# anilshanbhag/gpu-sort

Measured on AMD Instinct MI355X. Metric: Gkeys/s sorting 2^30 uint32 keys; achieved HBM GB/s vs roofline, higher is better.
Workload: dtype u32; 1 GPU; lsb_radix_sort_2^30_u32_uniform_keys_only; keys_per_gpu=1073741824, algorithm=lsb, distribution=uniform, parallelism=single

## Files before the change

### gpu-sort_amd/_lib.py

```python
import ctypes as C
import os

import torch

_HERE = os.path.dirname(os.path.abspath(__file__))
LIB_PATH = os.environ.get("GS_LIB_PATH", os.path.join(_HERE, "lib", "libgpusort.so"))
CSRC_DIR = os.path.join(_HERE, "csrc")
INCLUDE_DIR = os.path.join(os.path.dirname(_HERE), "include")

GS_KEY_U32, GS_KEY_I32, GS_KEY_F32, GS_KEY_U64, GS_KEY_I64, GS_KEY_F64 = 0, 1, 2, 3, 4, 5
GS_KEY_U8, GS_KEY_I8, GS_KEY_U16, GS_KEY_I16 = 6, 7, 8, 9
GS_KEY_F16, GS_KEY_BF16, GS_KEY_F8 = 10, 11, 12
GS_GEN_UNIFORM, GS_GEN_ZIPF, GS_GEN_ENTROPY_AND, GS_GEN_ENUMERATED = 0, 1, 2, 3

u64, i32, vp, sz = C.c_uint64, C.c_int, C.c_void_p, C.c_size_t
pp = C.POINTER(C.c_void_p)

SIGNATURES = {
    "gs_version": (i32, []),
    "gs_error_string": (C.c_char_p, [i32]),
    "gs_lsb_temp_bytes": (sz, [u64, i32]),
    "gs_lsb_sort_u32": (i32, [vp, sz, pp, pp, C.POINTER(i32), u64, i32, i32, i32, i32, vp]),
    "gs_lsb_copy_temp_bytes": (sz, [u64, i32]),
    "gs_lsb_sort_copy_u32": (i32, [vp, sz, vp, vp, vp, vp, u64, i32, i32, i32, i32, vp]),
    "gs_lsb_wide_temp_bytes": (sz, [u64, i32, i32]),
    "gs_lsb_sort_wide": (i32, [vp, sz, pp, pp, C.POINTER(i32), u64, i32, i32, i32, i32, i32, i32, vp]),
    "gs_lsb_any_temp_bytes": (sz, [u64, i32, i32]),
    "gs_lsb_sort_any": (i32, [vp, sz, vp, vp, vp, vp, u64, i32, i32, i32, i32, i32, vp]),
    "gs_lsb_narrow_temp_bytes": (sz, [u64, i32, i32]),
    "gs_lsb_sort_narrow": (i32, [vp, sz, vp, vp, vp, vp, u64, i32, i32, i32, i32, i32, vp]),
    "gs_lsb_narrow_tile": (C.c_uint32, [i32, i32]),
    "gs_lsb_geometry": (None, [u64, i32, C.POINTER(C.c_uint32), C.POINTER(C.c_uint32), C.POINTER(C.c_uint32)]),
    "gs_lsb_workspace_layout": (i32, [vp, u64, pp, pp, pp]),
    "gs_lsb_pipe_status": (i32, [vp, u64, C.POINTER(C.c_uint32), vp]),
    "gs_lsb_plan_status": (i32, [vp, u64, C.POINTER(C.c_uint32), vp]),
    "gs_lsb_plan_look_only": (i32, [vp, vp, vp, u64, i32, i32, vp]),
    "gs_lsb_plan_layout": (i32, [u64, C.POINTER(C.c_uint64)]),
    "gs_lsb_upsweep_u32": (i32, [vp, sz, vp, u64, i32, i32, i32, i32, vp]),
    "gs_lsb_scan_spine": (i32, [vp, sz, u64, vp]),
    "gs_lsb_downsweep_u32": (i32, [vp, sz, vp, vp, vp, vp, u64, i32, i32, i32, i32, i32, vp]),
    "gs_msb_temp_bytes": (sz, [u64, i32]),
    "gs_msb_sort_u32": (i32, [vp, sz, vp, vp, u64, vp, vp, pp, pp, i32, vp, i32]),
    "gs_msb_wide_temp_bytes": (sz, [u64, i32, i32]),
    "gs_msb_sort_wide": (i32, [vp, sz, vp, vp, u64, vp, vp, i32, i32, pp, pp, i32, vp, i32]),
    "gs_msb_large_temp_bytes": (sz, [u64, i32]),
    "gs_msb_sort_large_u32": (i32, [vp, sz, vp, vp, u64, vp, vp, i32, vp, i32]),
    "gs_msb_large_wide_temp_bytes": (sz, [u64, i32, i32]),
    "gs_msb_sort_large_wide": (i32, [vp, sz, vp, vp, u64, vp, vp, i32, i32, i32, vp, i32]),
    "gs_lsb_large_temp_bytes": (sz, [u64, i32, i32]),
    "gs_lsb_sort_large": (i32, [vp, sz, pp, pp, C.POINTER(i32), u64, i32, i32, i32, i32, i32, i32, vp]),
    "gs_lsb_narrow_large_temp_bytes": (sz, [u64, i32, i32]),
    "gs_lsb_sort_narrow_large": (i32, [vp, sz, vp, vp, vp, vp, u64, i32, i32, i32, i32, i32, vp]),
    "gs_topk_temp_bytes": (sz, [u64, u64, i32]),
    "gs_topk_u32": (i32, [vp, sz, vp, vp, vp, vp, u64, u64, i32, i32, vp]),
    "gs_topk_status": (i32, [vp, u64, u64, i32, C.POINTER(C.c_uint32), vp]),
    "gs_msb_census": (i32, [vp, u64, i32, vp, vp]),
    "gs_msb_wide_census": (i32, [vp, u64, i32, i32, vp, vp]),
    "gs_msb_capacities": (None, [u64, i32, C.POINTER(C.c_uint32), C.POINTER(C.c_uint32), C.POINTER(C.c_uint32)]),
    "gs_msb_classify_upto": (i32, [vp, sz, vp, vp, u64, i32, i32, vp]),
    "gs_msb_read_lists": (i32, [vp, u64, i32, i32, vp, C.c_uint32, C.POINTER(C.c_uint32), C.POINTER(C.POINTER(C.c_uint32)), C.c_uint32,
                                C.POINTER(C.c_uint32), vp]),
    "gs_segmented_temp_bytes": (sz, [u64, i32, C.c_uint32]),
    "gs_segmented_sort_u32": (i32, [vp, sz, pp, pp, C.POINTER(i32), u64, C.c_uint32, vp, vp, i32, i32, i32, i32, vp]),
    "gs_segmented_wide_temp_bytes": (sz, [u64, i32, i32, C.c_uint32]),
    "gs_segmented_sort_wide": (i32, [vp, sz, pp, pp, C.POINTER(i32), u64, C.c_uint32, vp, vp, i32, i32, i32, i32, i32, i32, vp]),
    "gs_segmented_narrow_temp_bytes": (sz, [u64, i32, i32, C.c_uint32]),
    "gs_segmented_sort_narrow": (i32, [vp, sz, pp, pp, C.POINTER(i32), u64, C.c_uint32, vp, vp, i32, i32, i32, i32, i32, vp]),
    "gs_segmented_narrow_cap": (C.c_uint32, [i32, i32]),
# ... 85 lines not shown
```

### gpu-sort_amd/csrc/gs_lsb_downsweep.inc

```
#ifndef GS_EXP_SLEEP_MODE
#define GS_EXP_SLEEP_MODE 0
#endif
#ifndef GS_EXP_SLEEP_MIN_TILES
#define GS_EXP_SLEEP_MIN_TILES 49152u
#endif
#ifndef GS_EXP_SLEEP_PAIRS
#define GS_EXP_SLEEP_PAIRS 0
#endif
template <bool HAS_VALUES, bool OFF64 = false>
struct DownsweepSmem {
    uint32_t whist[LSB_WAVES][RADIX];
#ifdef GS_EXP_ALLWAVE_KEYS
    uint16_t wbase[LSB_WAVES][RADIX];
#else
    uint16_t wbase[HAS_VALUES ? LSB_WAVES : 1][RADIX];
#endif
    std::conditional_t<OFF64, uint64_t, uint32_t> gbase[RADIX];
    uint32_t stage[LSB_TILE * (HAS_VALUES ? 2 : 1)];
    uint32_t dead;
};

#ifdef GS_EXP_PHASES
__device__ uint32_t gs_phase_buf[131072 * 16];
#define GS_PHASE(k)                                                                          \
    do {                                                                                     \
        const unsigned long long now_ = __builtin_amdgcn_s_memtime();                        \
        if (tid == 0 && t < 131072u) gs_phase_buf[t * 16 + (k)] = (uint32_t)(now_ - tprev_); \
        tprev_ = now_;                                                                       \
    } while (0)
#define GS_PHASE_WAIT(what) asm volatile("s_waitcnt " what ::: "memory")
#else
#define GS_PHASE(k) do { } while (0)
#define GS_PHASE_WAIT(what) do { } while (0)
#endif

constexpr uint32_t PIPE_SPIN_LIMIT = 1u << 18;

template <bool HAS_VALUES, bool TAIL, int TW, bool BIG, bool PIPE, bool OFF64 = false>
__device__ __forceinline__ void downsweep_tile(DownsweepSmem<HAS_VALUES, OFF64> &sm, const uint32_t t,
    const uint32_t *__restrict__ keys_in, uint32_t *__restrict__ keys_out, const uint32_t *__restrict__ vals_in,
    uint32_t *__restrict__ vals_out, const uint32_t *__restrict__ spine, const uint16_t *__restrict__ prefix16,
    const uint32_t *__restrict__ totals, const PassParams &p, const uint64_t *__restrict__ sc, uint32_t tag,
    uint32_t *__restrict__ error_word, const uint32_t tid_ = threadIdx.x, const uint64_t *__restrict__ dbase = nullptr)
{
#ifdef GS_EXP_ALLWAVE_KEYS
    constexpr bool ALLWAVE = true;
#else
    constexpr bool ALLWAVE = HAS_VALUES;
#endif

    [[maybe_unused]] const int tid = (int)tid_;
    const int lane = (int)(tid_ & 63u), w = (int)(tid_ >> 6);
    const uint32_t full_tiles = p.n / (uint32_t)LSB_TILE;
    auto tw_in = [&](uint32_t k) { return TW == 0 ? k : twiddle_in(k, TW == 2 ? p.f32_in : 0, p.xor_in); };
    auto tw_out = [&](uint32_t k) { return TW == 0 ? k : twiddle_out(k, TW == 2 ? p.f32_out : 0, p.xor_out); };
    uint32_t wbits = p.bits;
    asm volatile("" : "+v"(wbits));
    auto digit = [&](uint32_t k) { return __builtin_amdgcn_ubfe(k, p.shift, wbits); };

    uint32_t *my = sm.whist[w];
    const uint16_t *mybase = sm.wbase[w];
    const uint32_t wbase = (uint32_t)w * (WAVE * LSB_KPT) + lane;
    const uint32_t tail_valid = p.n - full_tiles * (uint32_t)LSB_TILE;
    (void)full_tiles;

#ifdef GS_EXP_PHASES
    unsigned long long tprev_ = __builtin_amdgcn_s_memtime();
    const unsigned long long t0_ = tprev_, r0_ = __builtin_amdgcn_s_memrealtime();
#endif
#ifdef GS_EXP_SLEEP_START
    __builtin_amdgcn_s_sleep(GS_EXP_SLEEP_START);
#endif
    if (!HAS_VALUES) __builtin_amdgcn_s_setprio(3);
    const uint64_t tile_base = (uint64_t)t * LSB_TILE;
    const uint32_t valid = TAIL ? tail_valid : (uint32_t)LSB_TILE;

    uint64_t scg[4] = {0, 0, 0, 0};
    const uint64_t *scrow = nullptr;
    if (PIPE && w == 0) {
        scrow = sc + (size_t)(t / LSB_CHUNK) * RADIX + 4 * lane;
#pragma unroll
        for (int q = 0; q < 4; ++q) scg[q] = ld_agent(scrow + q);
    }

    uint32_t key[LSB_KPT], val[HAS_VALUES ? LSB_KPT : 1], pos[LSB_KPT];
    {
        const uint32_t *kin = keys_in + tile_base;
        if (!TAIL) {
#pragma unroll
            for (int i = 0; i < LSB_KPT; ++i) key[i] = kin[wbase + i * WAVE];
        } else {
            const uint32_t pad = twiddle_out(0xffffffffu, TW == 2 ? p.f32_in : 0, TW ? p.xor_in : 0u);
#pragma unroll
            for (int i = 0; i < LSB_KPT; ++i) {
                const uint32_t idx = wbase + i * WAVE;
                key[i] = pad;
                if (idx < tail_valid) key[i] = kin[idx];
            }
        }
    }
    GS_PHASE(0);
#ifndef GS_EXP_RANK_PRIO
#define GS_EXP_RANK_PRIO 0
#endif
    if (!HAS_VALUES) __builtin_amdgcn_s_setprio(GS_EXP_RANK_PRIO);
    if (HAS_VALUES) {
        const uint32_t *vin = vals_in + tile_base;
#pragma unroll
        for (int i = 0; i < LSB_KPT; ++i) {
            const uint32_t idx = wbase + i * WAVE;
            val[i] = 0;
            if (!TAIL || idx < valid) val[i] = vin[idx];
        }
    }
    uint32_t dstart[4] = {0, 0, 0, 0};
    if constexpr (OFF64) {
        if (TAIL && w == 0) {
            const uint4 tot = reinterpret_cast<const uint4 *>(totals)[lane];
            dstart[0] = tot.x; dstart[1] = tot.y; dstart[2] = tot.z; dstart[3] = tot.w;
        }
    } else if (w == 0) {
        const uint4 tot = reinterpret_cast<const uint4 *>(totals)[lane];
        const uint32_t lane_sum = tot.x + tot.y + tot.z + tot.w;
        const uint32_t ex = wave_inclusive_scan(lane_sum) - lane_sum;
        dstart[0] = ex + (TAIL ? tot.x : 0u);
        dstart[1] = dstart[0] + (TAIL ? tot.y : tot.x);
        dstart[2] = dstart[1] + (TAIL ? tot.z : tot.y);
        dstart[3] = dstart[2] + (TAIL ? tot.w : tot.z);
    }

    uint32_t tbase[4] = {0, 0, 0, 0};
    if (!TAIL && !PIPE && w == 0) {
        const uint32_t *sp = spine + (uint32_t)(4 * lane) * p.grid + t / LSB_CHUNK;
        const uint2 pf = reinterpret_cast<const uint2 *>(prefix16 + (size_t)t * RADIX)[lane];
        tbase[0] = sp[0] + (pf.x & 0xffffu);
        tbase[1] = sp[p.grid] + (pf.x >> 16);
        tbase[2] = sp[2 * p.grid] + (pf.y & 0xffffu);
        tbase[3] = sp[3 * p.grid] + (pf.y >> 16);
    }

    if (PIPE && !TAIL && w == 0) {
        uint32_t spins = 0;
        bool gave_up = false;
        for (;;) {
            const bool ok = (uint32_t)(scg[0] >> 32) == tag && (uint32_t)(scg[1] >> 32) == tag &&
                            (uint32_t)(scg[2] >> 32) == tag && (uint32_t)(scg[3] >> 32) == tag;
            if (__builtin_amdgcn_ballot_w64(!ok) == 0) break;
            if (++spins > PIPE_SPIN_LIMIT) {
                if (lane == 0) atomicOr(error_word, 1u);
                gave_up = true;
                break;
            }
            __builtin_amdgcn_s_sleep(8);
#pragma unroll
            for (int q = 0; q < 4; ++q) scg[q] = ld_agent(scrow + q);
        }
        if (lane == 0) sm.dead = gave_up ? 1u : 0u;
        const uint64_t pf = ld_agent(reinterpret_cast<const uint64_t *>(prefix16 + (size_t)t * RADIX) + lane);
        tbase[0] = (uint32_t)scg[0] + (uint32_t)(pf & 0xffffu);
        tbase[1] = (uint32_t)scg[1] + (uint32_t)((pf >> 16) & 0xffffu);
        tbase[2] = (uint32_t)scg[2] + (uint32_t)((pf >> 32) & 0xffffu);
        tbase[3] = (uint32_t)scg[3] + (uint32_t)(pf >> 48);
    }

    auto publish_gbase = [&](const uint32_t (&ex)[4], const uint32_t (&run)[4]) {
// ... 21 lines not shown
            reinterpret_cast<uint4 *>(sm.gbase)[lane] = make_uint4(g[0], g[1], g[2], g[3]);
        }
    };

#pragma unroll
    for (int i = lane; i < RADIX; i += WAVE) my[i] = 0;
    GS_PHASE_WAIT("vmcnt(0)");
    GS_PHASE(1);
#pragma unroll
    for (int i = 0; i < LSB_KPT; ++i) key[i] = tw_in(key[i]);
    {
        uint32_t d_prev = 0, plo = 0, phi = 0;
#pragma unroll
        for (int i = 0; i <= LSB_KPT; ++i) {
            uint32_t d_cur = 0, clo = 0, chi = 0;
            if (i < LSB_KPT) {
                d_cur = digit(key[i]);
                match_digit(d_cur, clo, chi);
            }
            if (i > 0) {
                const uint32_t lower = count_lower(plo, phi);
                pos[i - 1] = my[d_prev] + lower;
                if (lower == 0)
                    __hip_atomic_fetch_add(&my[d_prev], (uint32_t)(__popc(plo) + __popc(phi)), __ATOMIC_RELAXED,
                                           __HIP_MEMORY_SCOPE_WAVEFRONT);
            }
            d_prev = d_cur; plo = clo; phi = chi;
        }
    }
#pragma unroll
    for (int i = 0; i < LSB_KPT; ++i) {
        asm volatile("" : "+v"(pos[i]), "+v"(key[i]));
    }
    GS_PHASE_WAIT("lgkmcnt(0)");
    GS_PHASE(2);
    __syncthreads();
    GS_PHASE(3);
    if (PIPE && !TAIL && sm.dead) return;

    if constexpr (ALLWAVE) {
        uint32_t run[4] = {0, 0, 0, 0}, below[4] = {0, 0, 0, 0};
#pragma unroll
        for (int j = 0; j < LSB_WAVES; ++j) {
            const uint4 x = reinterpret_cast<const uint4 *>(sm.whist[j])[lane];
            run[0] += x.x; run[1] += x.y; run[2] += x.z; run[3] += x.w;
            if (j < w) { below[0] += x.x; below[1] += x.y; below[2] += x.z; below[3] += x.w; }
        }
        const uint32_t lane_sum = run[0] + run[1] + run[2] + run[3];
        uint32_t ex[4];
        ex[0] = wave_inclusive_scan(lane_sum) - lane_sum;
        ex[1] = ex[0] + run[0];
        ex[2] = ex[1] + run[1];
        ex[3] = ex[2] + run[2];
        reinterpret_cast<uint2 *>(sm.wbase[w])[lane] =
            make_uint2((ex[0] + below[0]) | ((ex[1] + below[1]) << 16), (ex[2] + below[2]) | ((ex[3] + below[3]) << 16));
        if (w == 0) publish_gbase(ex, run);
    } else {
        if (w == 0) {
            uint32_t run[4] = {0, 0, 0, 0};
#pragma unroll
            for (int j = 0; j < LSB_WAVES; ++j) {
                const uint4 x = reinterpret_cast<const uint4 *>(sm.whist[j])[lane];
                run[0] += x.x; run[1] += x.y; run[2] += x.z; run[3] += x.w;
            }
            const uint32_t lane_sum = run[0] + run[1] + run[2] + run[3];
            uint32_t ex[4];
            ex[0] = wave_inclusive_scan(lane_sum) - lane_sum;
            ex[1] = ex[0] + run[0];
            ex[2] = ex[1] + run[1];
            ex[3] = ex[2] + run[2];
            publish_gbase(ex, run);
            asm volatile("" ::: "memory");
            uint4 e4 = make_uint4(ex[0] << 2, ex[1] << 2, ex[2] << 2, ex[3] << 2);
#pragma unroll
            for (int j = 0; j < LSB_WAVES; ++j) {
                const uint4 x = reinterpret_cast<const uint4 *>(sm.whist[j])[lane];
                reinterpret_cast<uint4 *>(sm.whist[j])[lane] = e4;
                e4.x += x.x << 2; e4.y += x.y << 2; e4.z += x.z << 2; e4.w += x.w << 2;
            }
        }
        __syncthreads();
    }
    GS_PHASE(4);

    {
        uint32_t wb[LSB_KPT];
#pragma unroll
        for (int i = 0; i < LSB_KPT; ++i) {
            const uint32_t d = digit(key[i]);
            wb[i] = ALLWAVE ? (uint32_t)mybase[d] : my[d];
        }
#pragma unroll
        for (int i = 0; i < LSB_KPT; ++i) {
            if (HAS_VALUES) {
                reinterpret_cast<uint2 *>(sm.stage)[pos[i] + wb[i]] = make_uint2(key[i], val[i]);
            } else if (ALLWAVE) {
                sm.stage[pos[i] + wb[i]] = key[i];
            } else {
                const uint32_t at = (pos[i] << 2) + wb[i];
                *reinterpret_cast<uint32_t *>(reinterpret_cast<char *>(sm.stage) + at) = key[i];
            }
        }
    }
    GS_PHASE_WAIT("lgkmcnt(0)");
    GS_PHASE(5);
    __syncthreads();
    GS_PHASE(6);
#ifndef GS_EXP_SLEEP
#define GS_EXP_SLEEP 32
#define GS_EXP_SLEEP_MODE_DEFAULT 0
#else
#define GS_EXP_SLEEP_MODE_DEFAULT GS_EXP_SLEEP_MODE
#endif
    if ((!HAS_VALUES || GS_EXP_SLEEP_PAIRS) && full_tiles >= GS_EXP_SLEEP_MIN_TILES) {
        [[maybe_unused]] const int ws = __builtin_amdgcn_readfirstlane(w);
#if GS_EXP_SLEEP_MODE_DEFAULT == 3
        if (ws & 1) __builtin_amdgcn_s_sleep(GS_EXP_SLEEP); else __builtin_amdgcn_s_sleep(GS_EXP_SLEEP_B);
#elif GS_EXP_SLEEP_MODE_DEFAULT == 4
        if (ws >= 4) __builtin_amdgcn_s_sleep(GS_EXP_SLEEP);
#elif GS_EXP_SLEEP_MODE_DEFAULT == 1
        if (ws & 1) __builtin_amdgcn_s_sleep(GS_EXP_SLEEP);
#elif GS_EXP_SLEEP_MODE_DEFAULT == 0
        __builtin_amdgcn_s_sleep(GS_EXP_SLEEP);
#endif
    }
#ifndef GS_EXP_STORE_PRIO
#define GS_EXP_STORE_PRIO 3
#endif
    if (!HAS_VALUES) __builtin_amdgcn_s_setprio(GS_EXP_STORE_PRIO);
#pragma unroll
    for (int i = 0; i < LSB_KPT; ++i) {
        const uint32_t slot = (uint32_t)w * (WAVE * LSB_KPT) + i * WAVE + lane;
        uint32_t k, v = 0;
// ... 41 lines not shown
```

### gpu-sort_amd/csrc/gs_lsb_plan.hip

```cpp
#include "gs_device.hpp"
#include "gs_lsb.hpp"
#include "gs_msb_tasks.hpp"
#ifndef GS_PLAN_N_MIN
#define GS_PLAN_N_MIN (1ull << 28)
#endif
#include <cstddef>
#include <cstdlib>
#include <cstring>
#include <type_traits>

namespace gs {

#include "gs_lsb_upsweep.inc"

#include "gs_lsb_downsweep.inc"

constexpr uint32_t PLAN_GROUPS = 65536;
constexpr uint32_t PLAN_WORDS = PLAN_GROUPS / 2;
constexpr uint32_t PLAN_PLANNED = 1u, PLAN_CLASSIC = 2u;
constexpr uint32_t PLAN_SKIP = 0xffffffffu;
constexpr int PLAN_LOOK_THREADS = 1024, PLAN_LOOK_WAVES = PLAN_LOOK_THREADS / WAVE, PLAN_LOOK_BATCH = 32;
constexpr uint32_t PLAN_LOOK_HALVES = PLAN_LOOK_WAVES / LSB_CHUNK;
static_assert(PLAN_LOOK_WAVES % LSB_CHUNK == 0, "a look workgroup takes whole chunks");
constexpr uint32_t PLAN_LOOK_MAX_GRID = MI355X_CUS;
constexpr uint32_t PLAN_BLOCKS = 128, PLAN_BLOCK_WORDS = PLAN_WORDS / PLAN_BLOCKS, PLAN_BLOCK_GROUPS = PLAN_GROUPS / PLAN_BLOCKS;
constexpr int PLAN_SORT_BITS = 16;
constexpr int PLAN_SKEW_LANES = 8;

struct PlanBlock {
    uint32_t route, max_group, nonempty, tasks[MSB_NCLASS], total;
    uint32_t shift[4];
    uint32_t ups_skip[4];
    MsbLevel level[2];
    uint32_t wg_bad[PLAN_LOOK_MAX_GRID];
    uint32_t blk_total[PLAN_BLOCKS], blk_max[PLAN_BLOCKS], blk_nonempty[PLAN_BLOCKS];
    uint32_t blk_class[PLAN_BLOCKS][MSB_NCLASS];
    uint32_t blk_class_base[PLAN_BLOCKS][MSB_NCLASS];
    uint32_t offsets[PLAN_GROUPS + 1];
};
static_assert(sizeof(MsbLevel) == 64 && offsetof(PlanBlock, level) == 64, "plan block layout");

__device__ __forceinline__ int plan_class_of(uint32_t size)
{
    return size <= msb_class_cap(0) ? 0 : size <= msb_class_cap(1) ? 1 : size <= msb_class_cap(2) ? 2 : 3;
}

__device__ __forceinline__ void look_add(uint32_t *tab, uint32_t *my, uint32_t g)
{
    const unsigned long long act = __builtin_amdgcn_ballot_w64(true);
    const uint32_t g0 = __builtin_amdgcn_readfirstlane(g);
    if (__builtin_amdgcn_ballot_w64(g == g0) == act) {
        if (count_lower_mask(act) == 0) {
            atomicAdd(&tab[g0 >> 1], (uint32_t)__popcll(act) << ((g0 & 1u) * 16u));
            atomicAdd(&my[g0 & 0xffu], (uint32_t)__popcll(act));
        }
    } else {
        atomicAdd(&tab[g >> 1], 1u << ((g & 1u) * 16u));
        atomicAdd(&my[g & 0xffu], 1u);
    }
}

__device__ __forceinline__ void look_add_skew(uint32_t *tab, uint32_t *my, uint32_t g, int lane)
{
    unsigned long long rest = ~0ull;
#pragma unroll
    for (int r = 0; r < 2; ++r) {
        if (rest == 0ull) break;
        const int lead = __builtin_amdgcn_readfirstlane(__builtin_ctzll(rest));
        const uint32_t g0 = (uint32_t)__builtin_amdgcn_readlane((int)g, lead);
        const unsigned long long m = __builtin_amdgcn_ballot_w64(g == g0) & rest;
        if (lane == lead) {
            atomicAdd(&tab[g0 >> 1], (uint32_t)__popcll(m) << ((g0 & 1u) * 16u));
// ... 115 lines not shown
    __syncthreads();
    if (tid == 0) plan->wg_bad[blockIdx.x] = sm.red[0] != sm.red[1] ? 1u : 0u;
}

__global__ __launch_bounds__(RADIX) void lsb_plan_reduce_kernel(const uint32_t *__restrict__ partial, PlanBlock *__restrict__ plan, uint32_t parts)
{
    __shared__ uint32_t scratch[8];
    __shared__ uint32_t red[2 + MSB_NCLASS];
    const uint32_t tid = threadIdx.x, wi = blockIdx.x * PLAN_BLOCK_WORDS + tid;
    if (tid < 2 + MSB_NCLASS) red[tid] = 0;
    uint32_t c0 = 0, c1 = 0;
#pragma unroll 8
    for (uint32_t g = 0; g < parts; ++g) {
        const uint32_t v = partial[(size_t)g * PLAN_WORDS + wi];
        c0 += v & 0xffffu;
        c1 += v >> 16;
    }
    uint32_t total = 0;
    const uint32_t ex = block_exclusive_scan_256(c0 + c1, scratch, &total);
    plan->offsets[2 * wi] = ex;
    plan->offsets[2 * wi + 1] = ex + c0;
    atomicMax(&red[0], c0 > c1 ? c0 : c1);
    if (c0) { atomicAdd(&red[1], 1u); atomicAdd(&red[2 + plan_class_of(c0)], 1u); }
    if (c1) { atomicAdd(&red[1], 1u); atomicAdd(&red[2 + plan_class_of(c1)], 1u); }
    __syncthreads();
    if (tid == 0) {
        plan->blk_total[blockIdx.x] = total;
        plan->blk_max[blockIdx.x] = red[0];
        plan->blk_nonempty[blockIdx.x] = red[1];
    }
    if (tid < MSB_NCLASS) plan->blk_class[blockIdx.x][tid] = red[2 + tid];
}

__global__ __launch_bounds__(RADIX) void lsb_plan_decide_kernel(PlanBlock *__restrict__ plan, uint32_t n, uint32_t parts)
{
    __shared__ uint32_t s_base, s_total, s_max, s_nz, s_cls[MSB_NCLASS], s_clsbase[MSB_NCLASS];
    const uint32_t tid = threadIdx.x, b = blockIdx.x;
    if (tid == 0) {
        uint32_t base = 0, total = 0, mx = 0, nz = 0;
        for (uint32_t i = 0; i < PLAN_BLOCKS; ++i) {
            if (i == b) base = total;
            total += plan->blk_total[i];
            const uint32_t m = plan->blk_max[i];
            mx = m > mx ? m : mx;
            nz += plan->blk_nonempty[i];
        }
        s_base = base; s_total = total; s_max = mx; s_nz = nz;
    } else if (tid <= MSB_NCLASS) {
        const uint32_t c = tid - 1u;
        uint32_t base = 0, total = 0;
        for (uint32_t i = 0; i < PLAN_BLOCKS; ++i) {
            if (i == b) base = total;
            total += plan->blk_class[i][c];
        }
        s_cls[c] = total; s_clsbase[c] = base;
    }
    const int any_bad = __syncthreads_or(tid < parts ? (int)plan->wg_bad[tid] : 0);
    const uint32_t g = b * PLAN_BLOCK_GROUPS + 2u * tid;
    plan->offsets[g] += s_base;
    plan->offsets[g + 1] += s_base;
    if (tid < MSB_NCLASS) plan->blk_class_base[b][tid] = s_clsbase[tid];
    if (b == 0 && tid == 0) {
        const bool planned = !any_bad && s_total == n && s_max <= msb_class_cap(MSB_NCLASS - 1);
        plan->route = planned ? PLAN_PLANNED : PLAN_CLASSIC;
        plan->max_group = s_max;
        plan->nonempty = s_nz;
        plan->total = s_total;
        MsbLevel l0{}, l1{};
        for (int c = 0; c < MSB_NCLASS; ++c) {
            plan->tasks[c] = planned ? s_cls[c] : 0u;
            l0.task_count[c] = planned ? s_cls[c] : 0u;
        }
        l0.keys = n;
        l1.packed = planned ? (1ull << 32) : 0ull;
        plan->level[0] = l0;
        plan->level[1] = l1;
        for (int q = 0; q < 4; ++q) {
            plan->shift[q] = planned ? (q < 2 ? 16u + 8u * (uint32_t)q : PLAN_SKIP) : 8u * (uint32_t)q;
            plan->ups_skip[q] = planned && q != 1 ? 1u : 0u;
        }
        plan->offsets[PLAN_GROUPS] = n;
    }
}

struct PlanLists { MsbTask *tasks[MSB_NCLASS]; uint32_t cap[MSB_NCLASS]; };
__global__ __launch_bounds__(PLAN_BLOCK_GROUPS) void lsb_plan_tasks_kernel(const PlanBlock *__restrict__ plan, PlanLists lists)
{
    __shared__ uint32_t wcnt[PLAN_BLOCK_GROUPS / WAVE][MSB_NCLASS];
    if (plan->route != PLAN_PLANNED) return;
    const uint32_t tid = threadIdx.x, g = blockIdx.x * PLAN_BLOCK_GROUPS + tid;
    const int w = wave_id(), lane = lane_id();
    const uint32_t off = plan->offsets[g], size = plan->offsets[g + 1] - off;
    const int cls = size ? plan_class_of(size) : -1;
    uint32_t lower = 0;
#pragma unroll
    for (int c = 0; c < MSB_NCLASS; ++c) {
        const unsigned long long m = __builtin_amdgcn_ballot_w64(cls == c);
        if (cls == c) lower = count_lower_mask(m);
        if (lane == 0) wcnt[w][c] = (uint32_t)__popcll(m);
    }
    __syncthreads();
    if (cls >= 0) {
        uint32_t idx = plan->blk_class_base[blockIdx.x][cls] + lower;
        for (int j = 0; j < w; ++j) idx += wcnt[j][cls];
        if (idx < lists.cap[cls]) lists.tasks[cls][idx] = MsbTask{off, size, (uint32_t)PLAN_SORT_BITS, 0u};
    }
}

template <bool PLAIN>
__global__ __launch_bounds__(LSB_THREADS, GS_EXP_UPS_WPE) void lsb_plan_upsweep_kernel(const uint32_t *__restrict__ keys,
                                                                       uint32_t *__restrict__ spine, uint16_t *__restrict__ prefix16,
                                                                       const uint32_t *__restrict__ slot_shift,
                                                                       const uint32_t *__restrict__ slot_ups_skip, PassParams p)
{
    __shared__ UpsweepSmem<false, false> sm;
    const uint32_t sh = *slot_shift;
    if (sh == PLAN_SKIP || *slot_ups_skip) return;
    p.shift = sh;
    upsweep_chunk<false, false, PLAIN>(sm, keys, chunk_of_block(blockIdx.x, p.grid), spine, prefix16, nullptr, nullptr, p, PipeParams{});
}

template <bool TAIL, int TW, bool BIG>
__global__ __launch_bounds__(LSB_THREADS, 6) void lsb_plan_downsweep_kernel(const uint32_t *__restrict__ keys_in, uint32_t *__restrict__ keys_out,
                                                                            const uint32_t *__restrict__ totals, const uint32_t *__restrict__ spine,
                                                                            const uint16_t *__restrict__ prefix16,
                                                                            const uint32_t *__restrict__ slot_shift, PassParams p)
{
    __shared__ __attribute__((aligned(16))) DownsweepSmem<false> sm;
    const uint32_t sh = *slot_shift;
    if (sh == PLAN_SKIP) return;
    p.shift = sh;
    const uint32_t full_tiles = p.n / (uint32_t)LSB_TILE;
    if (!TAIL && blockIdx.x >= full_tiles) return;
    const uint32_t t = TAIL ? full_tiles : tile_of_item_wide(blockIdx.x, full_tiles);
    downsweep_tile<false, TAIL, TW, BIG, false>(sm, t, keys_in, keys_out, nullptr, nullptr, spine, prefix16, totals, p, nullptr, 0u, nullptr);
}

static inline size_t align256(size_t x) { return (x + 255) & ~(size_t)255; }

static inline bool plan_enabled()
{
    static const bool v = [] { const char *e = getenv("GS_LSB_KEYS_PLAN"); return !(e && strcmp(e, "classic") == 0); }();
    return v;
}
constexpr uint64_t PLAN_N_MAX = (uint64_t)PLAN_GROUPS * 16620u;
constexpr uint64_t PLAN_N_FLOOR = 65536;
constexpr uint64_t PLAN_N_MIN = GS_PLAN_N_MIN;
static inline uint64_t plan_min_items()
{
    static const uint64_t v = [] {
        const char *e = getenv("GS_LSB_PLAN_MIN_ITEMS");
        if (!e) return PLAN_N_MIN;
        const uint64_t x = strtoull(e, nullptr, 10);
        return x < PLAN_N_FLOOR ? PLAN_N_FLOOR : x;
    }();
    return v;
}
static inline bool plan_has_block(uint64_t n) { return !lsb_pipe_enabled() && n >= plan_min_items(); }
static inline bool plan_size_ok(uint64_t n) { return plan_has_block(n) && n <= PLAN_N_MAX; }
static inline uint32_t plan_list_cap(uint64_t n, int c)
{
    const uint64_t m = c == 0 ? n : n / ((uint64_t)msb_class_cap(c - 1) + 1u) + 1u;
    return (uint32_t)(m < PLAN_GROUPS ? m : PLAN_GROUPS);
}
static inline size_t plan_lists_bytes(uint64_t n)
{
    size_t b = 0;
    for (int c = 0; c < MSB_NCLASS; ++c) b += (size_t)plan_list_cap(n, c) * sizeof(MsbTask);
    return b;
}
static inline size_t plan_block_offset(uint64_t n)
{
    const size_t a = lsb_temp_bytes(n), b = plan_lists_bytes(n);
    return align256(a > b ? a : b);
}
static inline size_t plan_temp_bytes(uint64_t n) { return plan_block_offset(n) + align256(sizeof(PlanBlock)); }

template <int TW, bool BIG>
static void launch_plan_downsweep(const uint32_t *kin, uint32_t *kout, const LsbWorkspace &ws, const uint32_t *slot_shift,
                                  const PassParams &p, hipStream_t s)
{
    hipLaunchKernelGGL((lsb_plan_downsweep_kernel<false, TW, BIG>), dim3(p.ds_grid), dim3(LSB_THREADS), 0, s, kin, kout, ws.totals,
                       ws.spine, ws.prefix16, slot_shift, p);
}

static int lsb_plan_slot(const uint32_t *kin, uint32_t *kout, const LsbWorkspace &ws, const uint32_t *slot_shift,
                         const uint32_t *slot_ups_skip, const PassParams &p, bool real, bool ups_real, hipStream_t s)
{
    {
        KernelTimer kt(ups_real ? GS_K_LSB_UPSWEEP : GS_K_OTHER, s);
        if (!p.f32_in && !p.xor_in)
            hipLaunchKernelGGL(lsb_plan_upsweep_kernel<true>, dim3(p.grid), dim3(LSB_THREADS), 0, s, kin, ws.spine, ws.prefix16, slot_shift,
                               slot_ups_skip, p);
        else
            hipLaunchKernelGGL(lsb_plan_upsweep_kernel<false>, dim3(p.grid), dim3(LSB_THREADS), 0, s, kin, ws.spine, ws.prefix16, slot_shift,
                               slot_ups_skip, p);
    }
    {
        if (const int e = lsb_scan_as(ws.spine, ws.totals, p.grid, s, real ? GS_K_LSB_SCAN : GS_K_OTHER)) return e;
    }
    {
        KernelTimer kt(real ? GS_K_LSB_DOWNSWEEP : GS_K_OTHER, s);
        if (p.n >= (uint32_t)LSB_TILE) {
            const int tw = (p.f32_in || p.f32_out) ? 2 : ((p.xor_in | p.xor_out) ? 1 : 0);
            const bool big = p.n > (1u << 30);
#define GS_PDS(TW_, BIG_) launch_plan_downsweep<TW_, BIG_>(kin, kout, ws, slot_shift, p, s)
            if (big) { if (tw == 2) GS_PDS(2, true); else if (tw == 1) GS_PDS(1, true); else GS_PDS(0, true); }
            else { if (tw == 2) GS_PDS(2, false); else if (tw == 1) GS_PDS(1, false); else GS_PDS(0, false); }
#undef GS_PDS
        }
        if (p.n % (uint32_t)LSB_TILE)
            hipLaunchKernelGGL((lsb_plan_downsweep_kernel<true, 2, true>), dim3(1), dim3(LSB_THREADS), 0, s, kin, kout, ws.totals,
                               (const uint32_t *)nullptr, (const uint16_t *)nullptr, slot_shift, p);
    }
    return (int)hipGetLastError();
}

static int lsb_plan_look(const uint32_t *keys, uint32_t *alt, const LsbWorkspace &ws, PlanBlock *plan, uint64_t n, const PassParams &tw,
                         hipStream_t s)
{
    const uint32_t parts = (uint32_t)(n / PLAN_WORDS < PLAN_LOOK_MAX_GRID ? n / PLAN_WORDS : PLAN_LOOK_MAX_GRID);
    const uint32_t chunks = lsb_make_params(n, 16, RADIX_BITS).grid;
    KernelTimer kt(GS_K_OTHER, s);
    hipLaunchKernelGGL(lsb_plan_look_kernel, dim3(parts), dim3(PLAN_LOOK_THREADS), 0, s, keys, alt, plan, ws.spine, ws.prefix16, (uint32_t)n,
                       chunks, tw.f32_in, tw.xor_in);
    hipLaunchKernelGGL(lsb_plan_reduce_kernel, dim3(PLAN_BLOCKS), dim3(RADIX), 0, s, alt, plan, parts);
    hipLaunchKernelGGL(lsb_plan_decide_kernel, dim3(PLAN_BLOCKS), dim3(RADIX), 0, s, plan, (uint32_t)n, parts);
    return (int)hipGetLastError();
}

int lsb_plan_sort(char *base, uint32_t *d_keys[2], int *selector, uint64_t n, int descending, int key_type, hipStream_t s)
{
    const LsbWorkspace ws = lsb_carve(base, n);
    char *lists_end = base + plan_block_offset(n);
    PlanBlock *plan = (PlanBlock *)lists_end;
    PlanLists lists;
    for (int c = MSB_NCLASS - 1; c >= 0; --c) {
        lists.cap[c] = plan_list_cap(n, c);
        lists_end -= (size_t)lists.cap[c] * sizeof(MsbTask);
        lists.tasks[c] = (MsbTask *)lists_end;
    }
    int sel = *selector, e;
    PassParams tw{};
    lsb_twiddle_masks(key_type, descending, true, true, tw);
    if ((e = lsb_plan_look(d_keys[sel], d_keys[sel ^ 1], ws, plan, n, tw, s))) return e;
    for (int slot = 0; slot < 4; ++slot) {
        PassParams p = lsb_make_params(n, 0, RADIX_BITS);
        lsb_twiddle_masks(key_type, descending, slot == 0, slot == 3, p);
        if ((e = lsb_plan_slot(d_keys[sel], d_keys[sel ^ 1], ws, &plan->shift[slot], &plan->ups_skip[slot], p, slot < 2, slot == 1, s))) return e;
        sel ^= 1;
    }
    {
        KernelTimer kt(GS_K_OTHER, s);
        hipLaunchKernelGGL(lsb_plan_tasks_kernel, dim3(PLAN_BLOCKS), dim3(PLAN_BLOCK_GROUPS), 0, s, plan, lists);
    }
    if ((e = (int)hipGetLastError())) return e;
    if ((e = msb_local_sorts_in_place(plan->level, lists.tasks, PLAN_GROUPS, PLAN_GROUPS, d_keys[sel], PLAN_SORT_BITS, n, tw.f32_out,
                                      tw.xor_out, s)))
        return e;
    *selector = sel;
    return hipSuccess;
}


bool lsb_plan_has_block(uint64_t n) { return plan_has_block(n); }
size_t lsb_plan_temp_bytes(uint64_t n) { return plan_temp_bytes(n); }
bool lsb_plan_applies(uint64_t n) { return plan_enabled() && plan_size_ok(n); }

}

using namespace gs;

extern "C" {

int gs_lsb_plan_status(void *d_temp, uint64_t num_items, uint32_t out[8], void *stream)
{
    GS_CLEAR_STALE_ERROR();
    if (!d_temp || !out || num_items >= (1ull << 32)) return hipErrorInvalidValue;
    memset(out, 0, 8 * sizeof(uint32_t));
    if (!plan_enabled() || !plan_size_ok(num_items)) return hipSuccess;
    const PlanBlock *plan = (const PlanBlock *)(gs_ws_base(d_temp) + plan_block_offset(num_items));
    hipError_t e = hipMemcpyAsync(out, plan, 8 * sizeof(uint32_t), hipMemcpyDeviceToHost, (hipStream_t)stream);
    if (e == hipSuccess) e = hipStreamSynchronize((hipStream_t)stream);
    return (int)e;
}

int gs_lsb_plan_look_only(void *d_temp, const void *d_keys, void *d_alt, uint64_t num_items, int key_type, int descending, void *stream)
{
    GS_CLEAR_STALE_ERROR();
    if (!d_temp || !d_keys || !d_alt || num_items >= (1ull << 32)) return hipErrorInvalidValue;
    if (!plan_enabled() || !plan_size_ok(num_items)) return hipErrorInvalidValue;
    char *base = gs_ws_base(d_temp);
    PassParams tw{};
    lsb_twiddle_masks(key_type, descending, true, true, tw);
    return lsb_plan_look((const uint32_t *)d_keys, (uint32_t *)d_alt, lsb_carve(base, num_items), (PlanBlock *)(base + plan_block_offset(num_items)),
                         num_items, tw, (hipStream_t)stream);
}

int gs_lsb_plan_layout(uint64_t num_items, uint64_t out[4])
{
    if (!out || num_items >= (1ull << 32) || !plan_enabled() || !plan_size_ok(num_items)) return hipErrorInvalidValue;
    char *base = (char *)(uintptr_t)GS_WS_ALIGN;
    const LsbWorkspace ws = lsb_carve(base, num_items);
    out[0] = (uint64_t)((char *)ws.spine - base);
    out[1] = (uint64_t)((char *)ws.prefix16 - base);
    out[2] = plan_block_offset(num_items);
    out[3] = lsb_make_params(num_items, 16, RADIX_BITS).grid;
    return hipSuccess;
}

}
```

### include/gpusort.h

```cpp
#ifndef GPUSORT_H_
#define GPUSORT_H_

#include <stddef.h>
#include <stdint.h>

#ifdef __cplusplus
extern "C" {
#endif

#define GS_VERSION 100

enum gs_key_type {
    GS_KEY_U32 = 0,
    GS_KEY_I32 = 1,
    GS_KEY_F32 = 2,
    GS_KEY_U64 = 3,
    GS_KEY_I64 = 4,
    GS_KEY_F64 = 5,
    GS_KEY_U8 = 6,
    GS_KEY_I8 = 7,
    GS_KEY_U16 = 8,
    GS_KEY_I16 = 9,
    GS_KEY_F16 = 10,
    GS_KEY_BF16 = 11,
    GS_KEY_F8 = 12
};

int         gs_version(void);
const char *gs_error_string(int err);


size_t gs_lsb_temp_bytes(uint64_t num_items, int has_values);

int gs_lsb_sort_u32(void *d_temp, size_t temp_bytes,
                    uint32_t *d_keys[2], uint32_t *d_vals[2], int *selector,
                    uint64_t num_items, int begin_bit, int end_bit,
                    int descending, int key_type, void *stream);

size_t gs_lsb_copy_temp_bytes(uint64_t num_items, int has_values);
int gs_lsb_sort_copy_u32(void *d_temp, size_t temp_bytes,
                         const uint32_t *d_keys_in, uint32_t *d_keys_out,
                         const uint32_t *d_vals_in, uint32_t *d_vals_out,
                         uint64_t num_items, int begin_bit, int end_bit,
                         int descending, int key_type, void *stream);

size_t gs_lsb_wide_temp_bytes(uint64_t num_items, int key_bytes, int val_bytes);
int gs_lsb_sort_wide(void *d_temp, size_t temp_bytes, void *d_keys[2], void *d_vals[2],
                     int *selector, uint64_t num_items, int key_bytes, int val_bytes,
                     int begin_bit, int end_bit, int descending, int key_type, void *stream);

void gs_lsb_geometry(uint64_t num_items, int has_values, uint32_t *grid, uint32_t *tile,
                     uint32_t *tiles_per_chunk);
int  gs_lsb_workspace_layout(void *d_temp, uint64_t num_items, uint32_t **d_spine,
                             uint32_t **d_totals, uint16_t **d_prefix16);
int  gs_lsb_pipe_status(void *d_temp, uint64_t num_items, uint32_t *h_status, void *stream);
int  gs_lsb_plan_status(void *d_temp, uint64_t num_items, uint32_t out[8], void *stream);
int  gs_lsb_plan_look_only(void *d_temp, const void *d_keys, void *d_alt, uint64_t num_items,
                           int key_type, int descending, void *stream);
int  gs_lsb_plan_layout(uint64_t num_items, uint64_t out[4]);
int  gs_lsb_upsweep_u32(void *d_temp, size_t temp_bytes, const uint32_t *d_keys_in,
                        uint64_t num_items, int shift, int bits, int descending,
                        int key_type_in, void *stream);
int  gs_lsb_scan_spine(void *d_temp, size_t temp_bytes, uint64_t num_items, void *stream);
int  gs_lsb_downsweep_u32(void *d_temp, size_t temp_bytes,
                          const uint32_t *d_keys_in, uint32_t *d_keys_out,
                          const uint32_t *d_vals_in, uint32_t *d_vals_out,
                          uint64_t num_items, int shift, int bits, int descending,
                          int key_type_in, int key_type_out, void *stream);

size_t gs_lsb_any_temp_bytes(uint64_t num_items, int key_type, int val_bytes);
int gs_lsb_sort_any(void *d_temp, size_t temp_bytes, const void *d_keys_in, void *d_keys_out,
                    const void *d_vals_in, void *d_vals_out, uint64_t num_items, int key_type, int val_bytes,
                    int begin_bit, int end_bit, int descending, void *stream);

size_t gs_lsb_narrow_temp_bytes(uint64_t num_items, int key_type, int val_bytes);
int gs_lsb_sort_narrow(void *d_temp, size_t temp_bytes, const void *d_keys_in, void *d_keys_out,
                       const void *d_vals_in, void *d_vals_out, uint64_t num_items, int key_type, int val_bytes,
                       int begin_bit, int end_bit, int descending, void *stream);
uint32_t gs_lsb_narrow_tile(int key_type, int val_bytes);


size_t gs_msb_temp_bytes(uint64_t num_items, int has_values);

int gs_msb_sort_u32(void *d_temp, size_t temp_bytes,
                    uint32_t *d_keys, uint32_t *d_vals, uint64_t num_items,
                    uint32_t *d_keys_alt, uint32_t *d_vals_alt,
                    uint32_t **d_sorted_keys, uint32_t **d_sorted_vals,
                    int key_type, void *stream, int synchronize);

// ... 127 lines not shown
```

Measured before the change: 147.5 Gkeys/s.

## Scatter second plan pass via per-digit-pair cursors instead of stable spine offsets

In the planned LSB path, the second pass can now run in a cursor mode. The plan's per-group offsets seed a cursor table, and each full tile whose keys share one upper digit claims output ranges with atomic adds instead of reading the spine/prefix bases. Tiles that straddle two upper digits, plus the tail, are listed and handled by a separate irregular kernel that scatters with wave-aggregated atomics. The upsweep for that pass is skipped in cursor mode, saving a full read of the keys, but the scatter loses stability within a tile group and adds atomic traffic and an extra launch.

```diff
diff --git a/gpu-sort_amd/_lib.py b/gpu-sort_amd/_lib.py
--- a/gpu-sort_amd/_lib.py
+++ b/gpu-sort_amd/_lib.py
@@ -34,6 +34,7 @@
     "gs_lsb_workspace_layout": (i32, [vp, u64, pp, pp, pp]),
     "gs_lsb_pipe_status": (i32, [vp, u64, C.POINTER(C.c_uint32), vp]),
     "gs_lsb_plan_status": (i32, [vp, u64, C.POINTER(C.c_uint32), vp]),
+    "gs_lsb_plan_cursor_status": (i32, [vp, u64, C.POINTER(C.c_uint32), vp]),
     "gs_lsb_plan_look_only": (i32, [vp, vp, vp, u64, i32, i32, vp]),
     "gs_lsb_plan_layout": (i32, [u64, C.POINTER(C.c_uint64)]),
     "gs_lsb_upsweep_u32": (i32, [vp, sz, vp, u64, i32, i32, i32, i32, vp]),
diff --git a/gpu-sort_amd/csrc/gs_lsb_downsweep.inc b/gpu-sort_amd/csrc/gs_lsb_downsweep.inc
--- a/gpu-sort_amd/csrc/gs_lsb_downsweep.inc
+++ b/gpu-sort_amd/csrc/gs_lsb_downsweep.inc
@@ -36,13 +36,15 @@
 
 constexpr uint32_t PIPE_SPIN_LIMIT = 1u << 18;
 
-template <bool HAS_VALUES, bool TAIL, int TW, bool BIG, bool PIPE, bool OFF64 = false>
+template <bool HAS_VALUES, bool TAIL, int TW, bool BIG, bool PIPE, bool OFF64 = false, bool CURSOR = false>
 __device__ __forceinline__ void downsweep_tile(DownsweepSmem<HAS_VALUES, OFF64> &sm, const uint32_t t,
     const uint32_t *__restrict__ keys_in, uint32_t *__restrict__ keys_out, const uint32_t *__restrict__ vals_in,
     uint32_t *__restrict__ vals_out, const uint32_t *__restrict__ spine, const uint16_t *__restrict__ prefix16,
     const uint32_t *__restrict__ totals, const PassParams &p, const uint64_t *__restrict__ sc, uint32_t tag,
-    uint32_t *__restrict__ error_word, const uint32_t tid_ = threadIdx.x, const uint64_t *__restrict__ dbase = nullptr)
+    uint32_t *__restrict__ error_word, const uint32_t tid_ = threadIdx.x, const uint64_t *__restrict__ dbase = nullptr,
+    uint32_t *__restrict__ cursor = nullptr, uint32_t *__restrict__ irr = nullptr, const uint32_t irr_cap = 0u)
 {
+    static_assert(!CURSOR || (!HAS_VALUES && !TAIL && !PIPE && !OFF64), "cursor mode: full tiles of keys-only three-launch passes");
 #ifdef GS_EXP_ALLWAVE_KEYS
     constexpr bool ALLWAVE = true;
 #else
@@ -99,6 +101,13 @@
             }
         }
     }
+    [[maybe_unused]] uint32_t cur_lo = 0, cur_hi = 0, claim[4] = {0, 0, 0, 0};
+    if constexpr (CURSOR) {
+        if (w == 0) {
+            cur_lo = (tw_in(keys_in[tile_base]) >> (p.shift - (uint32_t)RADIX_BITS)) & (uint32_t)(RADIX - 1);
+            cur_hi = (tw_in(keys_in[tile_base + (LSB_TILE - 1)]) >> (p.shift - (uint32_t)RADIX_BITS)) & (uint32_t)(RADIX - 1);
+        }
+    }
     GS_PHASE(0);
 #ifndef GS_EXP_RANK_PRIO
 #define GS_EXP_RANK_PRIO 0
@@ -119,7 +128,7 @@
             const uint4 tot = reinterpret_cast<const uint4 *>(totals)[lane];
             dstart[0] = tot.x; dstart[1] = tot.y; dstart[2] = tot.z; dstart[3] = tot.w;
         }
-    } else if (w == 0) {
+    } else if (!CURSOR && w == 0) {
         const uint4 tot = reinterpret_cast<const uint4 *>(totals)[lane];
         const uint32_t lane_sum = tot.x + tot.y + tot.z + tot.w;
         const uint32_t ex = wave_inclusive_scan(lane_sum) - lane_sum;
@@ -130,7 +139,7 @@
     }
 
     uint32_t tbase[4] = {0, 0, 0, 0};
-    if (!TAIL && !PIPE && w == 0) {
+    if (!TAIL && !PIPE && !CURSOR && w == 0) {
         const uint32_t *sp = spine + (uint32_t)(4 * lane) * p.grid + t / LSB_CHUNK;
         const uint2 pf = reinterpret_cast<const uint2 *>(prefix16 + (size_t)t * RADIX)[lane];
         tbase[0] = sp[0] + (pf.x & 0xffffu);
@@ -218,11 +227,22 @@
     for (int i = 0; i < LSB_KPT; ++i) {
         asm volatile("" : "+v"(pos[i]), "+v"(key[i]));
     }
+    if constexpr (CURSOR) {
+        if (w == 0 && lane == 0) {
+            const bool straddles = cur_lo != cur_hi;
+            sm.dead = straddles ? 1u : 0u;
+            if (straddles) {
+                const uint32_t at = atomicAdd(&irr[0], 1u);
+                if (at < irr_cap) irr[1u + at] = t;
+            }
+        }
+    }
     GS_PHASE_WAIT("lgkmcnt(0)");
     GS_PHASE(2);
     __syncthreads();
     GS_PHASE(3);
     if (PIPE && !TAIL && sm.dead) return;
+    if (CURSOR && sm.dead) return;
 
     if constexpr (ALLWAVE) {
         uint32_t run[4] = {0, 0, 0, 0}, below[4] = {0, 0, 0, 0};
@@ -255,7 +275,19 @@
             ex[1] = ex[0] + run[0];
             ex[2] = ex[1] + run[1];
             ex[3] = ex[2] + run[2];
-            publish_gbase(ex, run);
+            if constexpr (CURSOR) {
+                reinterpret_cast<uint4 *>(sm.gbase)[lane] = make_uint4(ex[0], ex[1], ex[2], ex[3]);
+                uint32_t *row = cursor + (size_t)__builtin_amdgcn_readfirstlane(cur_lo) * RADIX;
+#pragma unroll
+                for (int q = 0; q < 4; ++q) {
+                    const int d = q * WAVE + lane;
+                    const uint32_t e0 = sm.gbase[d], e1 = sm.gbase[d == RADIX - 1 ? d : d + 1];
+                    const uint32_t cnt = (d == RADIX - 1 ? (uint32_t)LSB_TILE : e1) - e0;
+                    claim[q] = __hip_atomic_fetch_add(row + d, cnt, __ATOMIC_RELAXED, __HIP_MEMORY_SCOPE_AGENT);
+                }
+            } else {
+                publish_gbase(ex, run);
+            }
             asm volatile("" ::: "memory");
             uint4 e4 = make_uint4(ex[0] << 2, ex[1] << 2, ex[2] << 2, ex[3] << 2);
 #pragma unroll
@@ -285,6 +317,16 @@
             } else {
                 const uint32_t at = (pos[i] << 2) + wb[i];
                 *reinterpret_cast<uint32_t *>(reinterpret_cast<char *>(sm.stage) + at) = key[i];
+            }
+        }
+    }
+    if constexpr (CURSOR) {
+        if (w == 0) {
+#pragma unroll
+            for (int q = 0; q < 4; ++q) {
+                const int d = q * WAVE + lane;
+                const uint32_t g = claim[q] - sm.gbase[d];
+                sm.gbase[d] = BIG ? g : g << 2;
             }
         }
     }
diff --git a/gpu-sort_amd/csrc/gs_lsb_plan.hip b/gpu-sort_amd/csrc/gs_lsb_plan.hip
--- a/gpu-sort_amd/csrc/gs_lsb_plan.hip
+++ b/gpu-sort_amd/csrc/gs_lsb_plan.hip
@@ -26,18 +26,25 @@
 constexpr uint32_t PLAN_BLOCKS = 128, PLAN_BLOCK_WORDS = PLAN_WORDS / PLAN_BLOCKS, PLAN_BLOCK_GROUPS = PLAN_GROUPS / PLAN_BLOCKS;
 constexpr int PLAN_SORT_BITS = 16;
 constexpr int PLAN_SKEW_LANES = 8;
+constexpr uint32_t PLAN_IRR_CAP = RADIX - 1;
+constexpr size_t PLAN_CURSOR_BYTES = (size_t)PLAN_GROUPS * sizeof(uint32_t);
 
 struct PlanBlock {
     uint32_t route, max_group, nonempty, tasks[MSB_NCLASS], total;
     uint32_t shift[4];
     uint32_t ups_skip[4];
     MsbLevel level[2];
-    uint32_t wg_bad[PLAN_LOOK_MAX_GRID];
+    union {
+        uint32_t wg_bad[PLAN_LOOK_MAX_GRID];
+        uint32_t irr[1 + PLAN_IRR_CAP];
+    };
     uint32_t blk_total[PLAN_BLOCKS], blk_max[PLAN_BLOCKS], blk_nonempty[PLAN_BLOCKS];
     uint32_t blk_class[PLAN_BLOCKS][MSB_NCLASS];
     uint32_t blk_class_base[PLAN_BLOCKS][MSB_NCLASS];
     uint32_t offsets[PLAN_GROUPS + 1];
+    uint32_t cursor_mode;
 };
+static_assert(1 + PLAN_IRR_CAP <= PLAN_LOOK_MAX_GRID, "the list of straddling tiles fits the look's flags");
 static_assert(sizeof(MsbLevel) == 64 && offsetof(PlanBlock, level) == 64, "plan block layout");
 
 __device__ __forceinline__ int plan_class_of(uint32_t size)
@@ -219,7 +226,7 @@
     if (tid < MSB_NCLASS) plan->blk_class[blockIdx.x][tid] = red[2 + tid];
 }
 
-__global__ __launch_bounds__(RADIX) void lsb_plan_decide_kernel(PlanBlock *__restrict__ plan, uint32_t n, uint32_t parts)
+__global__ __launch_bounds__(RADIX) void lsb_plan_decide_kernel(PlanBlock *__restrict__ plan, uint32_t n, uint32_t parts, uint32_t cursor_on)
 {
     __shared__ uint32_t s_base, s_total, s_max, s_nz, s_cls[MSB_NCLASS], s_clsbase[MSB_NCLASS];
     const uint32_t tid = threadIdx.x, b = blockIdx.x;
@@ -267,6 +274,7 @@
             plan->ups_skip[q] = planned && q != 1 ? 1u : 0u;
         }
         plan->offsets[PLAN_GROUPS] = n;
+        plan->cursor_mode = planned && cursor_on ? 1u : 0u;
     }
 }
 
@@ -323,11 +331,105 @@
     downsweep_tile<false, TAIL, TW, BIG, false>(sm, t, keys_in, keys_out, nullptr, nullptr, spine, prefix16, totals, p, nullptr, 0u, nullptr);
 }
 
+template <bool PLAIN>
+__global__ __launch_bounds__(LSB_THREADS, GS_EXP_UPS_WPE) void lsb_plan_upsweep2_kernel(const uint32_t *__restrict__ keys,
+                                                                        uint32_t *__restrict__ spine, uint16_t *__restrict__ prefix16,
+                                                                        PlanBlock *__restrict__ plan, uint32_t *__restrict__ cursor,
+                                                                        PassParams p)
+{
+    __shared__ UpsweepSmem<false, false> sm;
+    if (plan->cursor_mode) {
+        if (blockIdx.x == 0 && threadIdx.x == 0) plan->irr[0] = 0;
+        for (uint32_t i = blockIdx.x * (uint32_t)LSB_THREADS + threadIdx.x; i < PLAN_GROUPS; i += gridDim.x * (uint32_t)LSB_THREADS)
+            cursor[i] = plan->offsets[((i & (uint32_t)(RADIX - 1)) << RADIX_BITS) | (i >> RADIX_BITS)];
+        return;
+    }
+    const uint32_t sh = plan->shift[1];
+    if (sh == PLAN_SKIP || plan->ups_skip[1]) return;
+    p.shift = sh;
+    upsweep_chunk<false, false, PLAIN>(sm, keys, chunk_of_block(blockIdx.x, p.grid), spine, prefix16, nullptr, nullptr, p, PipeParams{});
+}
+
+template <bool TAIL, bool BIG>
+__global__ __launch_bounds__(LSB_THREADS, 6) void lsb_plan_scatter2_kernel(const uint32_t *__restrict__ keys_in, uint32_t *__restrict__ keys_out,
+                                                                           const uint32_t *__restrict__ totals, const uint32_t *__restrict__ spine,
+                                                                           const uint16_t *__restrict__ prefix16, PlanBlock *__restrict__ plan,
+                                                                           uint32_t *__restrict__ cursor, PassParams p)
+{
+    __shared__ __attribute__((aligned(16))) DownsweepSmem<false> sm;
+    const uint32_t sh = plan->shift[1];
+    if (sh == PLAN_SKIP) return;
+    p.shift = sh;
+    const uint32_t full_tiles = p.n / (uint32_t)LSB_TILE;
+    const uint32_t mode = plan->cursor_mode;
+    if constexpr (TAIL) {
+        if (mode) return;
+        downsweep_tile<false, true, 2, true, false>(sm, full_tiles, keys_in, keys_out, nullptr, nullptr, spine, prefix16, totals, p, nullptr, 0u,
+                                                    nullptr);
+    } else {
+        if (blockIdx.x >= full_tiles) return;
+        const uint32_t t = tile_of_item_wide(blockIdx.x, full_tiles);
+        if (mode)
+            downsweep_tile<false, false, 0, BIG, false, false, true>(sm, t, keys_in, keys_out, nullptr, nullptr, spine, prefix16, totals, p,
+                                                                     nullptr, 0u, nullptr, threadIdx.x, nullptr, cursor, plan->irr, PLAN_IRR_CAP);
+        else
+            downsweep_tile<false, false, 0, BIG, false>(sm, t, keys_in, keys_out, nullptr, nullptr, spine, prefix16, totals, p, nullptr, 0u,
+                                                        nullptr);
+    }
+}
+
+__global__ __launch_bounds__(LSB_THREADS) void lsb_plan_irregular_kernel(const uint32_t *__restrict__ keys_in, uint32_t *__restrict__ keys_out,
+                                                                         const PlanBlock *__restrict__ plan, uint32_t *__restrict__ cursor,
+                                                                         uint32_t n)
+{
+    if (!plan->cursor_mode) return;
+    const uint32_t full_tiles = n / (uint32_t)LSB_TILE;
+    uint32_t lo, len;
+    if (blockIdx.x == PLAN_IRR_CAP) {
+        lo = full_tiles * (uint32_t)LSB_TILE;
+        len = n - lo;
+    } else {
+        const uint32_t listed = plan->irr[0] < PLAN_IRR_CAP ? plan->irr[0] : PLAN_IRR_CAP;
+        if (blockIdx.x >= listed) return;
+        const uint32_t t = plan->irr[1u + blockIdx.x];
+        if (t >= full_tiles) return;
+        lo = t * (uint32_t)LSB_TILE;
+        len = (uint32_t)LSB_TILE;
+    }
+    const int lane = lane_id();
+    for (uint32_t i = threadIdx.x; i - (uint32_t)lane < len; i += (uint32_t)LSB_THREADS) {
+        const bool have = i < len;
+        const uint32_t k = have ? keys_in[lo + i] : 0u;
+        const uint32_t g = k >> 16, c = ((g & (uint32_t)(RADIX - 1)) << RADIX_BITS) | (g >> RADIX_BITS);
+        unsigned long long rest = __builtin_amdgcn_ballot_w64(have);
+        uint32_t at = 0;
+#pragma unroll
+        for (int r = 0; r < 2; ++r) {
+            if (rest == 0ull) break;
+            const int lead = __builtin_amdgcn_readfirstlane(__builtin_ctzll(rest));
+            const uint32_t c0 = (uint32_t)__builtin_amdgcn_readlane((int)c, lead);
+            const unsigned long long m = __builtin_amdgcn_ballot_w64(have && c == c0) & rest;
+            uint32_t first = 0;
+            if (lane == lead) first = __hip_atomic_fetch_add(cursor + c0, (uint32_t)__popcll(m), __ATOMIC_RELAXED, __HIP_MEMORY_SCOPE_AGENT);
+            first = (uint32_t)__builtin_amdgcn_readlane((int)first, lead);
+            if ((m >> lane) & 1ull) at = first + (uint32_t)__popcll(m & ((1ull << lane) - 1ull));
+            rest &= ~m;
+        }
+        if ((rest >> lane) & 1ull) at = __hip_atomic_fetch_add(cursor + c, 1u, __ATOMIC_RELAXED, __HIP_MEMORY_SCOPE_AGENT);
+        if (have && at < n) keys_out[at] = k;
+    }
+}
+
 static inline size_t align256(size_t x) { return (x + 255) & ~(size_t)255; }
 
 static inline bool plan_enabled()
 {
     static const bool v = [] { const char *e = getenv("GS_LSB_KEYS_PLAN"); return !(e && strcmp(e, "classic") == 0); }();
+    return v;
+}
+static inline bool plan_cursor_enabled()
+{
+    static const bool v = [] { const char *e = getenv("GS_LSB_PLAN_SCATTER2"); return !(e && strcmp(e, "stable") == 0); }();
     return v;
 }
 constexpr uint64_t PLAN_N_MAX = (uint64_t)PLAN_GROUPS * 16620u;
@@ -362,6 +464,7 @@
     return align256(a > b ? a : b);
 }
 static inline size_t plan_temp_bytes(uint64_t n) { return plan_block_offset(n) + align256(sizeof(PlanBlock)); }
+static inline uint32_t *plan_cursors(char *base, uint64_t n) { return (uint32_t *)(base + plan_block_offset(n) - PLAN_CURSOR_BYTES); }
 
 template <int TW, bool BIG>
 static void launch_plan_downsweep(const uint32_t *kin, uint32_t *kout, const LsbWorkspace &ws, const uint32_t *slot_shift,
@@ -371,6 +474,8 @@
                        ws.spine, ws.prefix16, slot_shift, p);
 }
 
+static int lsb_plan_slot2(const uint32_t *kin, uint32_t *kout, const LsbWorkspace &ws, PlanBlock *plan, uint32_t *cursor,
+                          const PassParams &p, hipStream_t s);
 static int lsb_plan_slot(const uint32_t *kin, uint32_t *kout, const LsbWorkspace &ws, const uint32_t *slot_shift,
                          const uint32_t *slot_ups_skip, const PassParams &p, bool real, bool ups_real, hipStream_t s)
 {
@@ -403,6 +508,38 @@
     return (int)hipGetLastError();
 }
 
+static int lsb_plan_slot2(const uint32_t *kin, uint32_t *kout, const LsbWorkspace &ws, PlanBlock *plan, uint32_t *cursor,
+                          const PassParams &p, hipStream_t s)
+{
+    if (p.f32_in || p.f32_out || p.xor_in || p.xor_out) return hipErrorInvalidValue;
+    if ((char *)cursor < (char *)ws.prefix16) return hipErrorInvalidValue;
+    {
+        KernelTimer kt(GS_K_OTHER, s);
+        hipLaunchKernelGGL(lsb_plan_upsweep2_kernel<true>, dim3(p.grid), dim3(LSB_THREADS), 0, s, kin, ws.spine, ws.prefix16, plan, cursor, p);
+    }
+    if (const int e = lsb_scan_as(ws.spine, ws.totals, p.grid, s, GS_K_LSB_SCAN)) return e;
+    {
+        KernelTimer kt(GS_K_LSB_DOWNSWEEP, s);
+        if (p.n >= (uint32_t)LSB_TILE) {
+            if (p.n > (1u << 30))
+                hipLaunchKernelGGL((lsb_plan_scatter2_kernel<false, true>), dim3(p.ds_grid), dim3(LSB_THREADS), 0, s, kin, kout, ws.totals,
+                                   ws.spine, ws.prefix16, plan, cursor, p);
+            else
+                hipLaunchKernelGGL((lsb_plan_scatter2_kernel<false, false>), dim3(p.ds_grid), dim3(LSB_THREADS), 0, s, kin, kout, ws.totals,
+                                   ws.spine, ws.prefix16, plan, cursor, p);
+        }
+        if (p.n % (uint32_t)LSB_TILE)
+            hipLaunchKernelGGL((lsb_plan_scatter2_kernel<true, true>), dim3(1), dim3(LSB_THREADS), 0, s, kin, kout, ws.totals,
+                               (const uint32_t *)nullptr, (const uint16_t *)nullptr, plan, cursor, p);
+    }
+    {
+        KernelTimer kt(GS_K_OTHER, s);
+        hipLaunchKernelGGL(lsb_plan_irregular_kernel, dim3(PLAN_IRR_CAP + (p.n % (uint32_t)LSB_TILE ? 1u : 0u)), dim3(LSB_THREADS), 0, s, kin,
+                           kout, plan, cursor, p.n);
+    }
+    return (int)hipGetLastError();
+}
+
 static int lsb_plan_look(const uint32_t *keys, uint32_t *alt, const LsbWorkspace &ws, PlanBlock *plan, uint64_t n, const PassParams &tw,
                          hipStream_t s)
 {
@@ -412,7 +549,7 @@
     hipLaunchKernelGGL(lsb_plan_look_kernel, dim3(parts), dim3(PLAN_LOOK_THREADS), 0, s, keys, alt, plan, ws.spine, ws.prefix16, (uint32_t)n,
                        chunks, tw.f32_in, tw.xor_in);
     hipLaunchKernelGGL(lsb_plan_reduce_kernel, dim3(PLAN_BLOCKS), dim3(RADIX), 0, s, alt, plan, parts);
-    hipLaunchKernelGGL(lsb_plan_decide_kernel, dim3(PLAN_BLOCKS), dim3(RADIX), 0, s, plan, (uint32_t)n, parts);
+    hipLaunchKernelGGL(lsb_plan_decide_kernel, dim3(PLAN_BLOCKS), dim3(RADIX), 0, s, plan, (uint32_t)n, parts, plan_cursor_enabled() ? 1u : 0u);
     return (int)hipGetLastError();
 }
 
@@ -434,7 +571,11 @@
     for (int slot = 0; slot < 4; ++slot) {
         PassParams p = lsb_make_params(n, 0, RADIX_BITS);
         lsb_twiddle_masks(key_type, descending, slot == 0, slot == 3, p);
-        if ((e = lsb_plan_slot(d_keys[sel], d_keys[sel ^ 1], ws, &plan->shift[slot], &plan->ups_skip[slot], p, slot < 2, slot == 1, s))) return e;
+        if (slot == 1 && plan_cursor_enabled())
+            e = lsb_plan_slot2(d_keys[sel], d_keys[sel ^ 1], ws, plan, plan_cursors(base, n), p, s);
+        else
+            e = lsb_plan_slot(d_keys[sel], d_keys[sel ^ 1], ws, &plan->shift[slot], &plan->ups_skip[slot], p, slot < 2, slot == 1, s);
+        if (e) return e;
         sel ^= 1;
     }
     {
@@ -472,6 +613,26 @@
     return (int)e;
 }
 
+int gs_lsb_plan_cursor_status(void *d_temp, uint64_t num_items, uint32_t out[4], void *stream)
+{
+    GS_CLEAR_STALE_ERROR();
+    if (!d_temp || !out || num_items >= (1ull << 32)) return hipErrorInvalidValue;
+    memset(out, 0, 4 * sizeof(uint32_t));
+    if (!plan_enabled() || !plan_size_ok(num_items)) return hipSuccess;
+    const PlanBlock *plan = (const PlanBlock *)(gs_ws_base(d_temp) + plan_block_offset(num_items));
+    uint32_t w[2] = {0, 0};
+    hipError_t e = hipMemcpyAsync(&w[0], &plan->cursor_mode, sizeof(uint32_t), hipMemcpyDeviceToHost, (hipStream_t)stream);
+    if (e == hipSuccess) e = hipMemcpyAsync(&w[1], &plan->irr[0], sizeof(uint32_t), hipMemcpyDeviceToHost, (hipStream_t)stream);
+    if (e == hipSuccess) e = hipStreamSynchronize((hipStream_t)stream);
+    if (e != hipSuccess) return (int)e;
+    if (w[0] == 1u) {
+        out[0] = 1;
+        out[2] = w[1];
+        out[1] = w[1] + (num_items % (uint64_t)LSB_TILE ? 1u : 0u);
+    }
+    return hipSuccess;
+}
+
 int gs_lsb_plan_look_only(void *d_temp, const void *d_keys, void *d_alt, uint64_t num_items, int key_type, int descending, void *stream)
 {
     GS_CLEAR_STALE_ERROR();
diff --git a/include/gpusort.h b/include/gpusort.h
--- a/include/gpusort.h
+++ b/include/gpusort.h
@@ -55,6 +55,7 @@
                              uint32_t **d_totals, uint16_t **d_prefix16);
 int  gs_lsb_pipe_status(void *d_temp, uint64_t num_items, uint32_t *h_status, void *stream);
 int  gs_lsb_plan_status(void *d_temp, uint64_t num_items, uint32_t out[8], void *stream);
+int  gs_lsb_plan_cursor_status(void *d_temp, uint64_t num_items, uint32_t out[4], void *stream);
 int  gs_lsb_plan_look_only(void *d_temp, const void *d_keys, void *d_alt, uint64_t num_items,
                            int key_type, int descending, void *stream);
 int  gs_lsb_plan_layout(uint64_t num_items, uint64_t out[4]);
```

After: 156.7 Gkeys/s, median of 6. 1.06x the previous value.
